# HasnainRaz/Fast-SRGAN

Measured on AMD Instinct MI355X. Metric: SR train-step images/sec (96->384 4x, full GAN step: G+D+VGG perceptual loss), higher is better.
Workload: dtype x3v; 1 GPU; BASELINE configs[2]: full GAN training step, 8 residual blocks / 64 filters, 96x96->384x384; per_gpu_batch=32, global_batch=32, parallelism=dp1, collectives=none, rccl_world_size=1, launch=hipGraph replay

## Files before the change

### fast-srgan_amd/csrc/conv_c3.hip

```cpp
#include "fsr_common.h"
#include "fsr_host.h"

namespace {

struct C3Args {
  const float* img;
  long long sn, sc, sh, sw;
  int N, H, W;
  float scale[3], shift[3];
  const void* wpk;
  const float* bias;
  const float* prelu;
  int act;
  float slope;
  int cout;
  void* out;
  void* preact;
  unsigned char* signs;
  const void* dz;
  float* ws;
  int tiles_x, tiles_y, tiles_per_slab, ntiles;
};

constexpr int PW = 18;
// ... 1 lines not shown
__device__ __forceinline__ int patch_off(int k) {
  const int tap = k / 3, ci = k - tap * 3;
  return ((tap / 3) * PW + (tap % 3)) * 3 + ci;
}

template <typename T> __device__ __forceinline__ float round_T(float v);
template <> __device__ __forceinline__ float round_T<float>(float v) { return v; }
template <> __device__ __forceinline__ float round_T<bf16_t>(float v) { return bf2f(f2bf(v)); }
template <> __device__ __forceinline__ float round_T<f16_t>(float v) { return (float)(f16_t)v; }

template <typename T, int TH>
__device__ __forceinline__ void stage_patch(const C3Args& a, float* patch, int n, int y0, int x0, int tid) {
  constexpr int PN = (TH + 2) * PW * 3;
  constexpr int PPT = (PN + 255) / 256;
  const float* src = a.img + n * a.sn;
  float v[PPT];
  unsigned okmask = 0u;
#pragma unroll
  for (int j = 0; j < PPT; ++j) {
    const int i = tid + j * 256;
    const int ci = i % 3, p = i / 3;
    const int px = p % PW, py = p / PW;
    const int y = y0 - 1 + py, x = x0 - 1 + px;
    const bool ok = i < PN && y >= 0 && y < a.H && x >= 0 && x < a.W;
    okmask |= (ok ? 1u : 0u) << j;
    v[j] = src[ok ? ci * a.sc + y * a.sh + x * a.sw : 0];
  }
#pragma unroll
  for (int j = 0; j < PPT; ++j) {
    const int i = tid + j * 256;
    const int ci = i % 3;
    const float sc = ci == 0 ? a.scale[0] : (ci == 1 ? a.scale[1] : a.scale[2]);
    const float sh = ci == 0 ? a.shift[0] : (ci == 1 ? a.shift[1] : a.shift[2]);
    if (i < PN) patch[i] = ((okmask >> j) & 1u) ? round_T<T>(v[j] * sc + sh) : 0.f;
  }
}

template <typename T, typename ST = T>
__global__ __launch_bounds__(256) void conv_c3_fwd_kernel(const C3Args a) {
  constexpr int TH = 16;
  __shared__ float patch[(TH + 2) * PW * 3];
  const int tid = threadIdx.x, lane = tid & 63, wave = __builtin_amdgcn_readfirstlane(tid >> 6);
  const int l15 = lane & 15, lg = lane >> 4;
  int bid = blockIdx.x;
  const int tx = bid % a.tiles_x;
  bid /= a.tiles_x;
  const int ty = bid % a.tiles_y;
  const int n = bid / a.tiles_y;
  const int nb = blockIdx.y;
  const int ntile = (a.cout - nb * 64 >= 64) ? 4 : (a.cout - nb * 64) / 16;
  stage_patch<T, TH>(a, patch, n, ty * TH, tx * 16, tid);

  const T* wpk = (const T*)a.wpk;
  int koff[8];
  if constexpr (sizeof(T) == 2) {
#pragma unroll
    for (int e = 0; e < 8; ++e) koff[e] = (8 * lg + e < 27) ? patch_off(8 * lg + e) : -1;
  } else {
#pragma unroll
    for (int j = 0; j < 8; ++j) koff[j] = (lg + 4 * j < 27) ? patch_off(lg + 4 * j) : -1;
  }
  constexpr bool X3 = std::is_same<ST, x3_t>::value;
  const bool wide = (sizeof(T) == 2 || X3) && ntile == 4;
  s16x8 wf16[4];
  float wf32[4][8];
#pragma unroll
  for (int t = 0; t < 4; ++t) {
    if (t < ntile) {
      const int ch = wide ? (t >> 1) * 32 + (l15 >> 2) * 8 + (t & 1) * 4 + (l15 & 3) : t * 16 + l15;
      const T* row = wpk + (size_t)(nb * 64 + ch) * 32;
      if constexpr (sizeof(T) == 2) {
        wf16[t] = *(const s16x8*)(row + 8 * lg);
      } else {
#pragma unroll
        for (int j = 0; j < 8; ++j) wf32[t][j] = row[lg + 4 * j];
      }
    }
  }
  float slope = (a.act == FSR_ACT_PRELU) ? a.prelu[0] : a.slope;
  if (a.act == FSR_ACT_NONE) slope = 1.f;
  if (a.act == FSR_ACT_RELU) slope = 0.f;
  __syncthreads();

  ST* outp = (ST*)a.out;
  ST* prep = (ST*)a.preact;
  const int gx = tx * 16 + l15;
  f32x4 bv[4];
#pragma unroll
  for (int i = 0; i < 4; ++i) bv[i] = (f32x4){0.f, 0.f, 0.f, 0.f};
  if (a.bias) {
    if (wide) {
#pragma unroll
      for (int p = 0; p < 2; ++p) {
        bv[2 * p] = *(const f32x4*)(a.bias + nb * 64 + p * 32 + lg * 8);
        bv[2 * p + 1] = *(const f32x4*)(a.bias + nb * 64 + p * 32 + lg * 8 + 4);
      }
    } else {
#pragma unroll
      for (int t = 0; t < 4; ++t)
        if (t < ntile) bv[t] = *(const f32x4*)(a.bias + nb * 64 + t * 16 + lg * 4);
    }
  }
#pragma unroll
  for (int m = 0; m < 4; ++m) {
    const int r = wave * 4 + m;
    const int gy = ty * TH + r;
    const float* base = patch + (r * PW + l15) * 3;
    float xv[8];
#pragma unroll
    for (int e = 0; e < 8; ++e) xv[e] = koff[e] >= 0 ? base[koff[e]] : 0.f;
    s16x8 xf16;
    if constexpr (sizeof(T) == 2) {
      const unsigned p0 = pack2<T>(xv[0], xv[1]), p1 = pack2<T>(xv[2], xv[3]);
      const unsigned p2 = pack2<T>(xv[4], xv[5]), p3 = pack2<T>(xv[6], xv[7]);
      xf16 = __builtin_bit_cast(s16x8, (u32x4){p0, p1, p2, p3});
    }
    if constexpr (sizeof(T) == 2) {
      if (wide) {
        f32x4 acc[4];
#pragma unroll
        for (int t = 0; t < 4; ++t) acc[t] = mfma16<T>(wf16[t], xf16, (f32x4){0.f, 0.f, 0.f, 0.f});
        if (gx < a.W && gy < a.H) {
          const size_t off = (((size_t)n * a.H + gy) * a.W + gx) * a.cout + nb * 64 + lg * 8;
#pragma unroll
          for (int p = 0; p < 2; ++p) {
            f32x4 lo = acc[2 * p], hi = acc[2 * p + 1];
            lo += bv[2 * p];
            hi += bv[2 * p + 1];
            if (prep)
              fsr_st<4>((u32x4*)((T*)prep + off + p * 32), (u32x4)((u32x4){pack2<T>(lo[0], lo[1]), pack2<T>(lo[2], lo[3]),
                                                       pack2<T>(hi[0], hi[1]), pack2<T>(hi[2], hi[3])}));
#pragma unroll
            for (int q = 0; q < 4; ++q) {
              lo[q] = fmaxf(lo[q], 0.f) + slope * fminf(lo[q], 0.f);
              hi[q] = fmaxf(hi[q], 0.f) + slope * fminf(hi[q], 0.f);
            }
            const u32x4 pk = (u32x4){pack2<T>(lo[0], lo[1]), pack2<T>(lo[2], lo[3]), pack2<T>(hi[0], hi[1]), pack2<T>(hi[2], hi[3])};
            fsr_st<4>((u32x4*)((T*)outp + off + p * 32), pk);
            if (a.signs) {
              unsigned b = 0u;
#pragma unroll
              for (int q = 0; q < 4; ++q) b |= ((int)(pk[q] << 16) > 0 ? 1u << (2 * q) : 0u) | ((int)(pk[q] & 0xffff0000u) > 0 ? 2u << (2 * q) : 0u);
              a.signs[(((size_t)n * a.H + gy) * a.W + gx) * (a.cout >> 3) + nb * 8 + p * 4 + lg] = (unsigned char)b;
            }
          }
        }
        continue;
      }
    }
    if constexpr (X3) {
      if (wide) {
        f32x4 acc[4];
#pragma unroll
        for (int t = 0; t < 4; ++t) {
          acc[t] = (f32x4){0.f, 0.f, 0.f, 0.f};
#pragma unroll
          for (int j = 0; j < 8; ++j) acc[t] = mfma_f32_16x16x4(wf32[t][j], xv[j], acc[t]);
        }
        if (gx < a.W && gy < a.H) {
          const size_t off = (((size_t)n * a.H + gy) * a.W + gx) * a.cout + nb * 64 + lg * 8;
#pragma unroll
          for (int p = 0; p < 2; ++p) {
            const f32x4 lo = acc[2 * p] + bv[2 * p], hi = acc[2 * p + 1] + bv[2 * p + 1];
            float v8[8] = {lo[0], lo[1], lo[2], lo[3], hi[0], hi[1], hi[2], hi[3]};
            if (prep) V16<x3_t, 4>::st((x3_t*)prep + off + p * 32, v8);
#pragma unroll
            for (int q = 0; q < 8; ++q) v8[q] = fmaxf(v8[q], 0.f) + slope * fminf(v8[q], 0.f);
            V16<x3_t, 4>::st((x3_t*)outp + off + p * 32, v8);
          }
        }
        continue;
      }
    }
    static_for<0, 4>([&](auto tc) {
      constexpr int t = decltype(tc)::value;
      if (t < ntile) {
        f32x4 acc = (f32x4){0.f, 0.f, 0.f, 0.f};
        if constexpr (sizeof(T) == 2) {
          acc = mfma16<T>(wf16[t], xf16, acc);
        } else {
#pragma unroll
          for (int j = 0; j < 8; ++j) acc = mfma_f32_16x16x4(wf32[t][j], xv[j], acc);
        }
        if (gx < a.W && gy < a.H) {
          const int co = nb * 64 + t * 16 + lg * 4;
          const size_t off = (((size_t)n * a.H + gy) * a.W + gx) * a.cout + co;
          acc += bv[t];
          if constexpr (sizeof(T) == 2) {
            if (prep) {
              u32x2 pk;
              pk.x = pack2<T>(acc[0], acc[1]);
              pk.y = pack2<T>(acc[2], acc[3]);
              fsr_st<4>((u32x2*)((T*)prep + off), (u32x2)(pk));
            }
          } else if constexpr (std::is_same<ST, x3_t>::value) {
            if (prep) x3_st4(prep + off, acc);
          } else {
            if (prep) *(f32x4*)(prep + off) = acc;
          }
#pragma unroll
          for (int q = 0; q < 4; ++q) acc[q] = fmaxf(acc[q], 0.f) + slope * fminf(acc[q], 0.f);
          if constexpr (sizeof(T) == 2) {
            u32x2 pk;
            pk.x = pack2<T>(acc[0], acc[1]);
            pk.y = pack2<T>(acc[2], acc[3]);
            fsr_st<4>((u32x2*)((T*)outp + off), (u32x2)(pk));
          } else if constexpr (std::is_same<ST, x3_t>::value) {
            x3_st4(outp + off, acc);
          } else {
            *(f32x4*)(outp + off) = acc;
          }
        }
      }
    });
  }
}

template <typename T, typename ST = T>
__global__ __launch_bounds__(256) void conv_c3_wgrad_kernel(const C3Args a) {
  constexpr int TH = 8;
  constexpr int PA = 64 + 16;
  __shared__ float patch[(TH + 2) * PW * 3];
  __shared__ __attribute__((aligned(16))) T dzt[TH * 16 * PA];
  const int tid = threadIdx.x, lane = tid & 63, wave = __builtin_amdgcn_readfirstlane(tid >> 6);
  const int l15 = lane & 15, lg = lane >> 4;
  const int slab = blockIdx.x, nb = blockIdx.y;
  const int cvalid = a.cout - nb * 64;
  const bool active = wave * 16 < cvalid;
  const ST* dzg = (const ST*)a.dz;
  constexpr int EPB = 16 / (int)sizeof(T);
  constexpr bool X3 = std::is_same<ST, x3_t>::value;

  const int off0 = patch_off(l15), off1 = (16 + l15 < 27) ? patch_off(16 + l15) : -1;
  const float ones27 = (l15 == 11) ? 1.f : 0.f;
  f32x4 acc0 = (f32x4){0.f, 0.f, 0.f, 0.f}, acc1 = (f32x4){0.f, 0.f, 0.f, 0.f};

  const int t0 = slab * a.tiles_per_slab;
  const int t1 = (t0 + a.tiles_per_slab < a.ntiles) ? t0 + a.tiles_per_slab : a.ntiles;
  for (int tile = t0; tile < t1; ++tile) {
    const int tx = tile % a.tiles_x;
    const int ty = (tile / a.tiles_x) % a.tiles_y;
    const int n = tile / (a.tiles_x * a.tiles_y);
    __syncthreads();
    stage_patch<T, TH>(a, patch, n, ty * TH, tx * 16, tid);
    if constexpr (X3) {
      constexpr int DU = TH * 16 * 8, DPT = DU / 256;
      u32x4 dh[DPT], dl[DPT];
#pragma unroll
      for (int j = 0; j < DPT; ++j) {
        const int u = tid + j * 256;
        const int unit = u % 8, p = u / 8;
        const int y = ty * TH + p / 16, x = tx * 16 + (p & 15);
        const bool ok = y < a.H && x < a.W && unit * 8 < cvalid;
        const char* hp = (const char*)x3_hi_ptr(dzg + (ok ? (((size_t)n * a.H + y) * a.W + x) * a.cout + nb * 64 + unit * 8 : 0));
        const u32x4 th = *(const u32x4*)hp, tl = *(const u32x4*)(hp + 64);
        dh[j] = ok ? th : (u32x4){0u, 0u, 0u, 0u};
        dl[j] = ok ? tl : (u32x4){0u, 0u, 0u, 0u};
      }
#pragma unroll
      for (int j = 0; j < DPT; ++j) {
        const int u = tid + j * 256;
        float* d = (float*)dzt + (u / 8) * PA + (u % 8) * 8;
        *(f32x4*)d = (f32x4){x3_join_lo(dh[j][0], dl[j][0]), x3_join_hi(dh[j][0], dl[j][0]), x3_join_lo(dh[j][1], dl[j][1]), x3_join_hi(dh[j][1], dl[j][1])};
        *(f32x4*)(d + 4) = (f32x4){x3_join_lo(dh[j][2], dl[j][2]), x3_join_hi(dh[j][2], dl[j][2]), x3_join_lo(dh[j][3], dl[j][3]), x3_join_hi(dh[j][3], dl[j][3])};
      }
    } else {
      constexpr int DU = TH * 16 * (64 / EPB), DPT = DU / 256;
      static_assert(DU % 256 == 0, "dz tile units per thread");
      u32x4 dv[DPT];
#pragma unroll
      for (int j = 0; j < DPT; ++j) {
        const int u = tid + j * 256;
        const int unit = u % (64 / EPB), p = u / (64 / EPB);
        const int y = ty * TH + p / 16, x = tx * 16 + (p & 15);
        const bool ok = y < a.H && x < a.W && unit * EPB < cvalid;
        const u32x4 t = *(const u32x4*)((const T*)dzg + (ok ? (((size_t)n * a.H + y) * a.W + x) * a.cout + nb * 64 + unit * EPB : 0));
        dv[j] = ok ? t : (u32x4){0u, 0u, 0u, 0u};
      }
#pragma unroll
      for (int j = 0; j < DPT; ++j) {
        const int u = tid + j * 256;
        *(u32x4*)(dzt + (u / (64 / EPB)) * PA + (u % (64 / EPB)) * EPB) = dv[j];
      }
    }
    __syncthreads();
    if (!active) continue;
    if constexpr (sizeof(T) == 2) {
      const int qrow = l15 >> 2, qch = (l15 & 3) * 4;
#pragma unroll
      for (int s = 0; s < TH / 2; ++s) {
        const int r = 2 * s + (lg >> 1), c0 = 8 * (lg & 1);
        const T* pa = dzt + (r * 16 + c0 + qrow) * PA + wave * 16 + qch;
        const s16x4 lo = __builtin_amdgcn_ds_read_tr16_b64_v4i16(FSR_LDS_PTR(s16x4, pa));
        const s16x4 hi = __builtin_amdgcn_ds_read_tr16_b64_v4i16(FSR_LDS_PTR(s16x4, pa + 4 * PA));
        const s16x8 af = (s16x8){lo[0], lo[1], lo[2], lo[3], hi[0], hi[1], hi[2], hi[3]};
        const float* pb = patch + (r * PW + c0) * 3;
        float b0[8], b1[8];
#pragma unroll
        for (int e = 0; e < 8; ++e) {
          b0[e] = pb[e * 3 + off0];
          b1[e] = off1 >= 0 ? pb[e * 3 + off1] : ones27;
        }
        const s16x8 bf0 = __builtin_bit_cast(s16x8, (u32x4){pack2<T>(b0[0], b0[1]), pack2<T>(b0[2], b0[3]),
                                                           pack2<T>(b0[4], b0[5]), pack2<T>(b0[6], b0[7])});
        const s16x8 bf1 = __builtin_bit_cast(s16x8, (u32x4){pack2<T>(b1[0], b1[1]), pack2<T>(b1[2], b1[3]),
                                                           pack2<T>(b1[4], b1[5]), pack2<T>(b1[6], b1[7])});
        acc0 = mfma16<T>(af, bf0, acc0);
        acc1 = mfma16<T>(af, bf1, acc1);
      }
    } else {
#pragma unroll 4
      for (int s = 0; s < TH * 4; ++s) {
        const int r = s >> 2, c = 4 * (s & 3) + lg;
        const float av = dzt[(r * 16 + c) * PA + wave * 16 + l15];
        const float* pb = patch + (r * PW + c) * 3;
        acc0 = mfma_f32_16x16x4(av, pb[off0], acc0);
        acc1 = mfma_f32_16x16x4(av, off1 >= 0 ? pb[off1] : ones27, acc1);
      }
    }
  }
  if (!active) return;
  float* o = a.ws + ((size_t)slab * a.cout + nb * 64 + wave * 16 + lg * 4) * 32 + l15;
#pragma unroll
  for (int r = 0; r < 4; ++r) {
    o[r * 32] = acc0[r];
    o[r * 32 + 16] = acc1[r];
  }
}

__global__ __launch_bounds__(256) void conv_c3_wgrad_reduce_kernel(const float* __restrict__ ws, float* __restrict__ dw, int nslab,
                                                                   int cout, float* __restrict__ dbias, int transposed) {
  __shared__ float red[8][32];
  const int total = cout * 32;
  const int k = threadIdx.x & 31, pl = threadIdx.x >> 5;
  const int co = blockIdx.x;
  const int i = co * 32 + k;
  float s = 0.f;
  const bool live = k < 27 || (k == 27 && dbias);
  if (live) {
    int j = pl;
    for (; j + 24 < nslab; j += 32) {
      const float v0 = ws[(size_t)j * total + i], v1 = ws[(size_t)(j + 8) * total + i];
      const float v2 = ws[(size_t)(j + 16) * total + i], v3 = ws[(size_t)(j + 24) * total + i];
      s = ((s + v0) + v1) + v2 + v3;
    }
    for (; j < nslab; j += 8) s += ws[(size_t)j * total + i];
  }
  red[pl][k] = s;
  __syncthreads();
  if (pl == 0 && live) {
    float r = red[0][k];
#pragma unroll
    for (int j = 1; j < 8; ++j) r += red[j][k];
    const int tap = k / 3, ci = k - tap * 3;
    float* o = (k == 27) ? dbias + co : (transposed ? dw + ((size_t)ci * cout + co) * 9 + (8 - tap) : dw + ((size_t)co * 3 + ci) * 9 + tap);
    *o += r;
  }
}

template <typename T>
__global__ void pack_c3_kernel(const float* __restrict__ w, T* __restrict__ out, int cout, int rows_pad, int transposed) {
  for (int i = blockIdx.x * blockDim.x + threadIdx.x; i < rows_pad * 32; i += gridDim.x * blockDim.x) {
    const int k = i & 31, row = i >> 5;
    float v = 0.f;
    if (row < cout && k < 27) {
      const int tap = k / 3, ci = k - tap * 3;
      v = transposed ? w[((size_t)ci * cout + row) * 9 + (8 - tap)] : w[((size_t)row * 3 + ci) * 9 + tap];
// ... 6 lines not shown
              long long sw, int n, int h, int w, const float (&scale3)[3], const float (&shift3)[3], int cout) {
  if (dtype != FSR_F32 && dtype != FSR_BF16 && dtype != FSR_F16 && dtype != FSR_X3) return fsr_fail(-2, "%s: unknown dtype %d", what, dtype);
  if (dtype == FSR_X3 && cout % 32) return fsr_fail(-2, "%s: x3 tensors have a multiple of 32 channels", what);
  if (!img) return fsr_fail(-1, "%s: null image", what);
  if (n <= 0 || h <= 0 || w <= 0) return fsr_fail(-2, "%s: bad dims", what);
  if (cout <= 0 || cout % 16) return fsr_fail(-2, "%s: cout=%d is not a multiple of 16", what, cout);
  if ((long long)n * h * w * cout >= (1LL << 31)) return fsr_fail(-2, "%s: tensors with 2^31 or more elements are not supported", what);
  a.img = img;
  a.sn = sn; a.sc = sc; a.sh = sh; a.sw = sw;
  a.N = n; a.H = h; a.W = w;
  for (int i = 0; i < 3; ++i) {
    a.scale[i] = scale3[i];
    a.shift[i] = shift3[i];
  }
  a.cout = cout;
  return 0;
}

}

extern "C" int fsr_pack_conv3x3_c3(int dtype, const float* w_oihw, int cout, void* packed, int transposed, fsr_stream_t stream_) {
  if (!w_oihw || !packed || cout <= 0) return fsr_fail(-1, "fsr_pack_conv3x3_c3: bad argument");
  const int rows_pad = (cout + 15) / 16 * 16;
  const int blocks = (rows_pad * 32 + 255) / 256;
  if (dtype == FSR_BF16)
    hipLaunchKernelGGL(pack_c3_kernel<bf16_t>, dim3(blocks), dim3(256), 0, (hipStream_t)stream_, w_oihw, (bf16_t*)packed, cout, rows_pad, transposed);
  else if (dtype == FSR_F16)
    hipLaunchKernelGGL(pack_c3_kernel<f16_t>, dim3(blocks), dim3(256), 0, (hipStream_t)stream_, w_oihw, (f16_t*)packed, cout, rows_pad, transposed);
  else if (dtype == FSR_F32 || dtype == FSR_X3)
    hipLaunchKernelGGL(pack_c3_kernel<float>, dim3(blocks), dim3(256), 0, (hipStream_t)stream_, w_oihw, (float*)packed, cout, rows_pad, transposed);
  else
    return fsr_fail(-2, "fsr_pack_conv3x3_c3: unknown dtype %d", dtype);
  return fsr_check_launch("pack_c3_kernel");
}

extern "C" int fsr_conv3x3_c3_fwd(int dtype, const float* img, long long sn, long long sc, long long sh, long long sw, int n,
                                  int h, int w, float scale0, float scale1, float scale2, float shift0, float shift1,
                                  float shift2, const void* packed_w, const float* bias, int act, float slope, const float* prelu_weight, int cout, void* out,
                                  void* preact, void* signs, fsr_stream_t stream_) {
  C3Args a = {};
  const float scale3[3] = {scale0, scale1, scale2}, shift3[3] = {shift0, shift1, shift2};
  if (int rc = fill_args(a, "fsr_conv3x3_c3_fwd", dtype, img, sn, sc, sh, sw, n, h, w, scale3, shift3, cout)) return rc;
  if (!packed_w || !out) return fsr_fail(-1, "fsr_conv3x3_c3_fwd: null argument");
  if (act == FSR_ACT_PRELU && !prelu_weight) return fsr_fail(-1, "fsr_conv3x3_c3_fwd: PReLU needs its weight");
  if (act == FSR_ACT_TANH) return fsr_fail(-2, "fsr_conv3x3_c3_fwd: tanh is not a first-layer activation");
  a.wpk = packed_w;
  a.bias = bias;
  a.prelu = prelu_weight;
  a.act = act;
  a.slope = slope;
  a.out = out;
  a.preact = preact;
  if (dtype == FSR_X3 && ((((size_t)out | (size_t)preact) & 127) != 0)) return fsr_fail(-2, "fsr_conv3x3_c3_fwd: x3 tensors must be 128-byte aligned");
  if (signs && (dtype == FSR_F32 || dtype == FSR_X3 || cout % 64 != 0)) return fsr_fail(-2, "fsr_conv3x3_c3_fwd: sign bits are written by the 16-bit kernels for cout %% 64 == 0");
  a.signs = (unsigned char*)signs;
  a.tiles_x = (w + 15) / 16;
  a.tiles_y = (h + 15) / 16;
  const long long nwg = (long long)a.tiles_x * a.tiles_y * n;
  if (nwg > 0x7fffffffLL) return fsr_fail(-2, "fsr_conv3x3_c3_fwd: bad grid");
  const dim3 grid((unsigned)nwg, (unsigned)((cout + 63) / 64));
  if (dtype == FSR_BF16) hipLaunchKernelGGL(conv_c3_fwd_kernel<bf16_t>, grid, dim3(256), 0, (hipStream_t)stream_, a);
  else if (dtype == FSR_F16) hipLaunchKernelGGL(conv_c3_fwd_kernel<f16_t>, grid, dim3(256), 0, (hipStream_t)stream_, a);
  else if (dtype == FSR_X3) hipLaunchKernelGGL((conv_c3_fwd_kernel<float, x3_t>), grid, dim3(256), 0, (hipStream_t)stream_, a);
  else hipLaunchKernelGGL(conv_c3_fwd_kernel<float>, grid, dim3(256), 0, (hipStream_t)stream_, a);
  return fsr_check_launch("conv_c3_fwd_kernel");
}

static int c3_wgrad_slabs(int n, int h, int w, int* tiles_x, int* tiles_y, int* per) {
  *tiles_x = (w + 15) / 16;
  *tiles_y = (h + 7) / 8;
  const long long ntiles = (long long)*tiles_x * *tiles_y * n;
  long long want = 1024;
  if (want > ntiles) want = ntiles;
  *per = (int)((ntiles + want - 1) / want);
  return (int)((ntiles + *per - 1) / *per);
}

extern "C" size_t fsr_conv3x3_c3_wgrad_workspace(int n, int h, int w, int cout) {
  int tx, ty, per;
  if (n <= 0 || h <= 0 || w <= 0 || cout <= 0) return 0;
  return (size_t)c3_wgrad_slabs(n, h, w, &tx, &ty, &per) * cout * 32 * sizeof(float);
}

extern "C" int fsr_conv3x3_c3_wgrad(int dtype, const float* img, long long sn, long long sc, long long sh, long long sw,
                                    int n, int h, int w, float scale0, float scale1, float scale2, float shift0,
                                    float shift1, float shift2, const void* dz, int cout, float* dw_oihw, float* dbias, void* workspace, int transposed,
                                    fsr_stream_t stream_) {
  C3Args a = {};
  const float scale3[3] = {scale0, scale1, scale2}, shift3[3] = {shift0, shift1, shift2};
  if (int rc = fill_args(a, "fsr_conv3x3_c3_wgrad", dtype, img, sn, sc, sh, sw, n, h, w, scale3, shift3, cout)) return rc;
  if (!dz || !dw_oihw || !workspace) return fsr_fail(-1, "fsr_conv3x3_c3_wgrad: null argument");
  if (dtype == FSR_X3 && (((size_t)dz & 127) != 0)) return fsr_fail(-2, "fsr_conv3x3_c3_wgrad: x3 tensors must be 128-byte aligned");
  a.dz = dz;
  a.ws = (float*)workspace;
  const int nslab = c3_wgrad_slabs(n, h, w, &a.tiles_x, &a.tiles_y, &a.tiles_per_slab);
  a.ntiles = a.tiles_x * a.tiles_y * n;
  const dim3 grid((unsigned)nslab, (unsigned)((cout + 63) / 64));
  if (dtype == FSR_BF16) hipLaunchKernelGGL(conv_c3_wgrad_kernel<bf16_t>, grid, dim3(256), 0, (hipStream_t)stream_, a);
  else if (dtype == FSR_F16) hipLaunchKernelGGL(conv_c3_wgrad_kernel<f16_t>, grid, dim3(256), 0, (hipStream_t)stream_, a);
  else if (dtype == FSR_X3) hipLaunchKernelGGL((conv_c3_wgrad_kernel<float, x3_t>), grid, dim3(256), 0, (hipStream_t)stream_, a);
  else hipLaunchKernelGGL(conv_c3_wgrad_kernel<float>, grid, dim3(256), 0, (hipStream_t)stream_, a);
  if (int rc = fsr_check_launch("conv_c3_wgrad_kernel")) return rc;
  hipLaunchKernelGGL(conv_c3_wgrad_reduce_kernel, dim3(cout), dim3(256), 0, (hipStream_t)stream_, (const float*)workspace,
                     dw_oihw, nslab, cout, dbias, transposed);
  return fsr_check_launch("conv_c3_wgrad_reduce_kernel");
}
```

### fast-srgan_amd/csrc/conv_s2d3.hip

```cpp
#include "fsr_common.h"
#include "fsr_conv_args.h"
#include "fsr_host.h"

#include <stdlib.h>

#ifndef FSR_ABLS
#define FSR_ABLS 0
#endif

namespace {

constexpr int S2D_ABL = FSR_ABLS;

typedef float f32x16 __attribute__((ext_vector_type(16)));

template <typename T> struct Mfma32;
template <> struct Mfma32<bf16_t> {
  static __device__ __forceinline__ f32x16 run(s16x8 a, s16x8 b, f32x16 c) {
    return __builtin_amdgcn_mfma_f32_32x32x16_bf16(__builtin_bit_cast(bf16x8_hw, a), __builtin_bit_cast(bf16x8_hw, b), c, 0, 0, 0);
  }
};
template <> struct Mfma32<f16_t> {
  static __device__ __forceinline__ f32x16 run(s16x8 a, s16x8 b, f32x16 c) {
    return __builtin_amdgcn_mfma_f32_32x32x16_f16(__builtin_bit_cast(f16x8_hw, a), __builtin_bit_cast(f16x8_hw, b), c, 0, 0, 0);
// ... 343 lines not shown
          if (ok1) fsr_st<16>((u32x4*)((T*)outp + off1), o1);
        }
        }
      });
    });
    if (!has_nxt) break;
    cur = nxt;
#pragma unroll
    for (int k = 0; k < HPW; ++k) hv_cur[k] = hv_nxt[k];
    ws_cur = ws_nxt;
    tile = next;
    next = tile + nround;
    has_nxt = next < a.t3_ntiles;
    acc_zero();
  }
}

int s2d_cus() {
  if (const char* e = getenv("FSR_PERSIST_CUS")) {
    const int v = atoi(e);
    if (v > 0) return v;
  }
  static int cus = 0;
  if (cus == 0) {
    int dev = 0;
    hipDeviceProp_t prop;
    cus = (hipGetDevice(&dev) == hipSuccess && hipGetDeviceProperties(&prop, dev) == hipSuccess && prop.multiProcessorCount > 0)
              ? prop.multiProcessorCount : 256;
  }
  return cus;
}

template <typename T, bool X3 = false>
int s2d_launch(ConvKArgs& a, hipStream_t stream) {
  auto kern = conv_s2d3_kernel<T, X3>;
  static bool attr_set = false;
  if (!attr_set) {
    (void)hipFuncSetAttribute((const void*)kern, hipFuncAttributeMaxDynamicSharedMemorySize, S2D_LDS);
    attr_set = true;
  }
  long long grid = (long long)s2d_cus() * 2;
  if (grid > a.t3_ntiles) grid = a.t3_ntiles;
  hipLaunchKernelGGL(kern, dim3((unsigned)grid), dim3(S2D_NW * 64), S2D_LDS, stream, a);
  fsr_note_kernel("conv_s2d3_kernel<%s>", X3 ? "x3" : (std::is_same<T, f16_t>::value ? "f16" : "bf16"));
  const int rc = fsr_check_launch("conv_s2d3_kernel");
  return rc ? rc : 1;
}

}

int fsr_conv_s2d3_try(int dtype, ConvKArgs& a, hipStream_t stream) {
  static const bool off = getenv("FSR_S2D3") && atoi(getenv("FSR_S2D3")) == 0;
  if (off || (dtype != FSR_BF16 && dtype != FSR_F16 && dtype != FSR_X3)) return 0;
  if (dtype == FSR_X3 && ((a.Cin & 63) != 0 || (a.Cin >> 6) * 3 >= (1 << 15) || a.dmask_bits)) return 0;
  if (a.Cin < 64 || a.Cin % 32 != 0 || a.Cout % 64 != 0 || a.Cout < 64 || a.CoutPad != a.Cout) return 0;
  if (a.ps || a.in_ps || a.out_f32 || a.preact || a.oscale || a.bias || a.stats || a.pool2 || a.act != FSR_ACT_NONE || a.dmask_add) return 0;
  if (a.IH != (a.FOH - 1) / 2 + 1 || a.IW != (a.FOW - 1) / 2 + 1) return 0;
  if ((long long)a.N * a.IH * a.IW * a.Cin >= (1LL << 31) || (long long)a.N * a.FOH * a.FOW * a.Cout >= (1LL << 31)) return 0;
  ConvKArgs b = a;
  b.tiles_x = (b.IW + 15) / 16;
  b.tiles_y = (b.IH + S2D_TH - 1) / S2D_TH;
  b.nblk_n = b.Cout / S2D_BN;
  const long long ntiles = (long long)b.tiles_x * b.tiles_y * b.N * b.nblk_n;
  if (ntiles <= 0 || ntiles > 0x7fffffffLL) return 0;
  b.t3_ntiles = (int)ntiles;
  const int want = b.Cin >= 128 ? S2D_BN : 0;
  if (b.query) {
    a.wlin_want = want;
    return 1;
  }
  if (b.wlin != 0 && b.wlin != S2D_BN)
    return fsr_fail(-2, "conv_s2d3: the filter pack is stage-contiguous in blocks of %d channels, this launch needs %d", b.wlin, S2D_BN);
  for (int t = 0; t < 9; ++t) b.t3_woff[t] = b.wlin ? (unsigned)(t * S2D_BN * 64) : (unsigned)((size_t)t * b.CoutPad * b.Cin * 2);
  const int rc = dtype == FSR_X3 ? s2d_launch<bf16_t, true>(b, stream) : (dtype == FSR_F16 ? s2d_launch<f16_t>(b, stream) : s2d_launch<bf16_t>(b, stream));
  if (rc == 1) a = b;
  return rc;
}
```

### fast-srgan_amd/csrc/fsr_api.hip

```cpp
#include <string.h>

#include "fsr_common.h"
#include "fsr_conv_args.h"
#include "fsr_host.h"

static thread_local char g_err[512] = "";

int fsr_fail(int code, const char* fmt, ...) {
  va_list ap;
  va_start(ap, fmt);
  vsnprintf(g_err, sizeof(g_err), fmt, ap);
  va_end(ap);
  return code;
}

int fsr_check_launch(const char* what) {
  hipError_t e = hipGetLastError();
  if (e != hipSuccess) return fsr_fail(-3, "%s: launch failed: %s", what, hipGetErrorString(e));
  return 0;
}

static thread_local char g_kernel[160] = "";

void fsr_note_kernel(const char* fmt, ...) {
// ... 31 lines not shown
static int conv3x3_enqueue(const fsr_conv_desc* d, ConvKArgs& a, hipStream_t stream);

static int conv3x3_impl(const fsr_conv_desc* d, const void* in, const void* packed_w, const float* bias,
                        const float* prelu_weight, const float* oscale, const void* dact_mask, float dact_slope,
                        void* out, void* preact, float* stats, void* scratch, hipStream_t stream, int* query_block);

extern "C" int fsr_conv3x3(const fsr_conv_desc* d, const void* in, const void* packed_w, const float* bias,
                           const float* prelu_weight, const float* oscale, const void* dact_mask, float dact_slope,
                           void* out, void* preact, float* stats, void* scratch, fsr_stream_t stream_) {
  return conv3x3_impl(d, in, packed_w, bias, prelu_weight, oscale, dact_mask, dact_slope, out, preact, stats, scratch,
                      (hipStream_t)stream_, nullptr);
}

extern "C" int fsr_conv3x3_pack_block(const fsr_conv_desc* d, int optional_tensors) {
  if (!d) return fsr_fail(-1, "fsr_conv3x3_pack_block: null descriptor");
  static const float dummy_f[4] = {0.f, 0.f, 0.f, 0.f};
  const void* some = dummy_f;
  fsr_conv_desc q = *d;
  q.pack_lin = 0;
  int block = 0;
  const int rc = conv3x3_impl(&q, some, some, (optional_tensors & FSR_OPT_BIAS) ? dummy_f : nullptr,
                              (optional_tensors & FSR_OPT_PRELU) ? dummy_f : nullptr, (optional_tensors & FSR_OPT_OSCALE) ? dummy_f : nullptr,
                              (optional_tensors & FSR_OPT_MASK) ? some : nullptr, 0.f, (void*)some,
                              (optional_tensors & FSR_OPT_PREACT) ? (void*)some : nullptr,
                              (optional_tensors & FSR_OPT_STATS) ? (float*)some : nullptr,
                              (optional_tensors & FSR_OPT_STATS) ? (void*)some : nullptr, nullptr, &block);
  return rc < 0 ? rc : block;
}

static int conv3x3_impl(const fsr_conv_desc* d, const void* in, const void* packed_w, const float* bias,
                        const float* prelu_weight, const float* oscale, const void* dact_mask, float dact_slope,
                        void* out, void* preact, float* stats, void* scratch, hipStream_t stream, int* query_block) {
  if (!d || !in || !packed_w || !out) return fsr_fail(-1, "fsr_conv3x3: null argument");
  if (stats && !scratch) return fsr_fail(-1, "fsr_conv3x3: statistics need the scratch buffer (fsr_conv3x3_scratch bytes)");
  if (d->stride != 1 && d->stride != 2) return fsr_fail(-2, "fsr_conv3x3: stride must be 1 or 2");
  if (d->act == FSR_ACT_PRELU && !prelu_weight) return fsr_fail(-1, "fsr_conv3x3: PReLU needs its weight");
  if (d->n <= 0 || d->ih <= 0 || d->iw <= 0 || d->oh <= 0 || d->ow <= 0) return fsr_fail(-2, "fsr_conv3x3: bad dims");

  ConvKArgs a;
  memset(&a, 0, sizeof(a));
  a.in = in;
  a.wpk = packed_w;
  a.out = out;
  a.bias = bias;
  a.prelu = prelu_weight;
  a.preact = preact;
  a.oscale = oscale;
  a.dmask = dact_mask;
  a.dmask_slope = dact_slope;
  a.dmask_add = (dact_mask && d->mask_is_addend == 1) ? 1 : 0;
  a.dmask_bits = (dact_mask && d->mask_is_addend == 2) ? 1 : 0;
  if (d->mask_is_addend && !dact_mask) return fsr_fail(-1, "fsr_conv3x3: mask_is_addend needs the dact_mask tensor");
  if (d->mask_is_addend < 0 || d->mask_is_addend > 2) return fsr_fail(-2, "fsr_conv3x3: mask_is_addend must be 0, 1 or 2");
  if (a.dmask_bits && (d->mode != FSR_CONV_DGRAD || d->stride != 2 || d->dtype == FSR_F32 || d->dtype == FSR_X3 || d->cout % 64 != 0))
    return fsr_fail(-2, "fsr_conv3x3: a sign-bit mask (mask_is_addend = 2) is read by the stride-2 data gradients of the 16-bit modes, cout %% 64 == 0");
  a.stats = stats ? (float*)scratch : nullptr;
  a.stats_P_max = stats ? (int)stats_slots_bound(d) : 0;
  a.query = query_block ? 1 : 0;
  a.wlin = d->pack_lin;
  if (d->pack_lin != 0 && d->pack_lin != 64 && d->pack_lin != 128) return fsr_fail(-2, "fsr_conv3x3: pack_lin must be 0, 64 or 128");
  a.N = d->n;
  a.IH = d->ih;
  a.IW = d->iw;
  a.Cin = d->dtype == FSR_X3 ? 2 * d->cin : d->cin;
  a.Cout = d->cout;
  if (d->dtype == FSR_X3) {
    if (d->cin % 32 != 0) return fsr_fail(-2, "fsr_conv3x3: x3 tensors have a multiple of 32 channels (cin = %d)", d->cin);
    if (!d->out_f32 && d->cout % 32 != 0) return fsr_fail(-2, "fsr_conv3x3: x3 tensors have a multiple of 32 channels (cout = %d)", d->cout);
    if (d->pixel_shuffle && (d->cout / 4) % 32 != 0) return fsr_fail(-2, "fsr_conv3x3: x3 pixel shuffle needs cout / 4 %% 32 == 0");
    if (d->in_pixel_shuffled && (d->cin / 4) % 32 != 0) return fsr_fail(-2, "fsr_conv3x3: x3 in_pixel_shuffled needs cin / 4 %% 32 == 0");
    if (!query_block && ((((size_t)in | (d->out_f32 ? 0 : (size_t)out) | (size_t)preact | (size_t)dact_mask) & 127) != 0))
      return fsr_fail(-2, "fsr_conv3x3: x3 tensors must be 128-byte aligned");
  }
  a.CoutPad = (d->cout + 15) / 16 * 16;
  a.FOH = d->oh;
  a.FOW = d->ow;
  a.act = d->act;
  a.slope = d->slope;
  a.ps = d->pixel_shuffle;
  a.in_ps = d->in_pixel_shuffled;
  a.out_f32 = d->out_f32;
  a.pool2 = d->pool2;
  if (d->pool2 && (d->mode != FSR_CONV_FWD || d->dtype == FSR_F32 || d->stride != 1 || d->pixel_shuffle || d->out_f32 || stats || preact ||
                   dact_mask || oscale || (d->oh & 1) || (d->ow & 1) || d->cout % 16 != 0 || d->act == FSR_ACT_TANH))
    return fsr_fail(-2, "fsr_conv3x3: pool2 is for stride-1 forward launches of the 16-bit modes with even output extents "
                        "(no statistics / pre-activation / mask / scale tensors, no pixel shuffle)");
  if (d->out_f32 < 0 || d->out_f32 > FSR_OUT_I420) return fsr_fail(-2, "fsr_conv3x3: unknown output kind %d", d->out_f32);
  if (d->out_f32 == FSR_OUT_U8 && (d->act != FSR_ACT_TANH || d->cout > 16 || d->pixel_shuffle || d->mode != FSR_CONV_FWD))
    return fsr_fail(-2, "fsr_conv3x3: uint8 image output is for tanh heads (forward, cout <= 16)");
  if (d->out_f32 == FSR_OUT_I420) {
    if (d->act != FSR_ACT_TANH || d->cout != 3 || d->pixel_shuffle || d->mode != FSR_CONV_FWD || d->stride != 1 || stats || preact ||
        dact_mask || oscale)
      return fsr_fail(-2, "fsr_conv3x3: I420 output is for 3-channel tanh heads (forward, stride 1, no pixel shuffle, no statistics / "
                          "pre-activation / mask / scale tensors)");
    if ((d->oh & 1) || (d->ow & 1)) return fsr_fail(-2, "fsr_conv3x3: I420 output needs even output extents (%d x %d)", d->oh, d->ow);
    if ((d->yuv_matrix != FSR_YUV_BT601 && d->yuv_matrix != FSR_YUV_BT709) || (d->yuv_full_range != 0 && d->yuv_full_range != 1))
      return fsr_fail(-2, "fsr_conv3x3: I420 output: unknown colour matrix %d / range %d", d->yuv_matrix, d->yuv_full_range);
  }
  a.yuv_matrix = d->yuv_matrix;
  a.yuv_full = d->yuv_full_range;
  if (a.ps && stats) return fsr_fail(-2, "fsr_conv3x3: statistics are not available together with pixel shuffle");
  if ((stats || preact || dact_mask) && (d->cout % 16 != 0 || (d->out_f32 && d->dtype != FSR_F32)))
    return fsr_fail(-2, "fsr_conv3x3: statistics / pre-activation / mask tensors need cout %% 16 == 0 and a `dtype` output");
  if (a.ps && (d->cout % 16 != 0)) return fsr_fail(-2, "fsr_conv3x3: pixel shuffle needs cout %% 16 == 0");
  if (a.in_ps && (d->cin % 4 != 0)) return fsr_fail(-2, "fsr_conv3x3: in_pixel_shuffled needs cin %% 4 == 0");
  if (stats && d->mode == FSR_CONV_DGRAD && d->stride != 1)
    return fsr_fail(-2, "fsr_conv3x3: statistics are not available for stride-2 data gradients");

  if (int rc = conv3x3_enqueue(d, a, stream)) return rc;
  if (query_block) {
    *query_block = a.wlin_want;
    return 0;
  }
  if (stats) {
    return fsr_launch_reduce_partials((const float*)scratch, stats, d->n, a.stats_P, d->cout * 2, d->cout * 2, a.stats_tpi, a.stats_per, 1.f, 0, stream);
  }
  return 0;
}

static int conv3x3_enqueue(const fsr_conv_desc* d, ConvKArgs& a, hipStream_t stream) {
  if (d->mode == FSR_CONV_FWD) {
    if (d->oh != (d->ih - 1) / d->stride + 1 || d->ow != (d->iw - 1) / d->stride + 1)
      return fsr_fail(-2, "fsr_conv3x3: output dims do not match k=3,p=1,stride=%d", d->stride);
    a.GH = d->oh;
// ... 75 lines not shown
```

### fast-srgan_amd/ops.py

```python
import ctypes
import os
import weakref

import torch

from . import _lib as L

_DT = {"f32": (L.FSR_F32, torch.float32, 16), "bf16": (L.FSR_BF16, torch.bfloat16, 32), "f16": (L.FSR_F16, torch.float16, 32),
       "x3": (L.FSR_X3, torch.float32, 32)}


class Compute:

    def __init__(self, name="f16"):
        if name not in _DT:
            raise ValueError("compute dtype must be 'bf16', 'f16', 'x3' or 'f32', got %r" % (name,))
        self.name = name
        self.code, self.torch_dtype, self.cpad = _DT[name]
        self.x3 = name == "x3"
        self.pack_dtype = torch.bfloat16 if self.x3 else self.torch_dtype
        self.pack_kmul = 2 if self.x3 else 1
        self.is16 = name in ("bf16", "f16")

    def pad(self, c):
# ... 431 lines not shown
    prof = PROFILE_CONV
    if prof is not None:
        ev0, ev1 = torch.cuda.Event(enable_timing=True), torch.cuda.Event(enable_timing=True)
        ev0.record()
    L.check(L.lib().fsr_conv3x3_wgrad(ctypes.byref(d), _p(x), _p(dy), _p(dw), _p(ws), _stream()), "fsr_conv3x3_wgrad")
    if prof is not None:
        ev1.record()
        nbytes = x.numel() * x.element_size() + dy.numel() * dy.element_size() + cout * cin * 9 * 4
        prof.append((ev0, ev1, 2.0 * n * oh * ow * cout * cin * 9, nbytes, "conv_wgrad_kernel", "wgrad"))
    return dw


def image_to_nhwc(cd, img, scale=(1.0, 1.0, 1.0), shift=(0.0, 0.0, 0.0)):
    _check_dev(img)
    if img.dtype != torch.float32:
        img = img.float()
    n, c, h, w = img.shape
    if c != 3:
        raise ValueError("expected a 3-channel image batch, got %s" % (tuple(img.shape),))
    out = _empty((n, h, w, cd.cpad), cd.torch_dtype, img.device)
    sn, sc, sh, sw = img.stride()
    L.check(L.lib().fsr_image_to_nhwc(cd.code, _p(img), sn, sc, sh, sw, n, h, w, scale[0], scale[1], scale[2], shift[0],
                                      shift[1], shift[2], _p(out), cd.cpad, _stream()), "fsr_image_to_nhwc")
    return out


class ConvCfg:

    def __init__(self, cd, *, stride=1, act=L.ACT_NONE, slope=0.0, pixel_shuffle=False, stats=False, image_in=False,
                 in_scale=(1.0, 1.0, 1.0), in_shift=(0.0, 0.0, 0.0), tanh_head=False, input_act_bwd=None,
                 act_bwd_by_consumer=False, u8_head=False, pool_after=False, n_alias=0, emit_signs=False, i420_head=None):
        self.input_act_bwd, self.act_bwd_by_consumer = input_act_bwd, act_bwd_by_consumer
        self.cd, self.stride, self.act, self.slope = cd, stride, act, slope
        self.pixel_shuffle, self.stats, self.image_in = pixel_shuffle, stats, image_in
        self.in_scale, self.in_shift, self.tanh_head = in_scale, in_shift, tanh_head
        self.u8_head = u8_head and tanh_head
        self.i420_head = i420_head if tanh_head else None
        self.pool_after = pool_after
        self.n_alias = n_alias
        self.emit_signs = emit_signs


class Conv3x3Fn(torch.autograd.Function):

    @staticmethod
    def forward(ctx, x, weight, bias, prelu, cfg, grad_on=True):
        ctx.grad_on = grad_on
        cd = cfg.cd
        cout, cin = weight.shape[0], weight.shape[1]
        if (cfg.image_in and cfg.stride == 1 and cout % 16 == 0 and not (cfg.pixel_shuffle or cfg.stats or cfg.tanh_head)
                and USE_C3_KERNELS):
            return Conv3x3Fn._forward_c3(ctx, x, weight, bias, prelu, cfg)
        ctx.c3 = False
        ctx.in_signs = getattr(x, "_fsr_signs", None) if (cfg.input_act_bwd is not None and cfg.stride == 2 and cd.is16) else None
        if cfg.image_in:
            xin = image_to_nhwc(cd, x, cfg.in_scale, cfg.in_shift)
        else:
            xin = x if x.is_contiguous() else x.contiguous()
            if xin.dtype != cd.torch_dtype:
                raise L.FsrError("activation dtype %s does not match the module's compute dtype %s" % (xin.dtype, cd.name))
        cin_pad = xin.shape[3]
        wpk = FilterSpec(weight, L.PACK_FWD_PS if cfg.pixel_shuffle else L.PACK_FWD, cin_pad)
        training = ctx.grad_on and any(ctx.needs_input_grad)
        if (cfg.u8_head or cfg.i420_head or cfg.pool_after) and training:
            raise L.FsrError("the uint8 / I420 head and fused max-pool epilogues are inference-only: they have no gradient")
        act = L.ACT_TANH if cfg.tanh_head else cfg.act
        want_pre = training and act == L.ACT_PRELU
        b32 = bias if bias is None or bias.dtype == torch.float32 else bias.float()
        out, pre, stats = conv3x3_raw(cd, xin, wpk, cout, stride=cfg.stride, bias=b32, act=act, slope=cfg.slope,
                                      prelu=prelu, pixel_shuffle=cfg.pixel_shuffle, out_f32=cfg.tanh_head,
                                      want_stats=cfg.stats, want_preact=want_pre, alg_k=cin, out_u8=cfg.u8_head,
                                      pool2=cfg.pool_after, out_i420=cfg.i420_head)
        ctx.cfg = cfg
        ctx.dims = (cout, cin, tuple(xin.shape))
        ctx.has_bias = bias is not None
        ctx.x_is_image = cfg.image_in
        saved_act = pre if want_pre else (out if act in (L.ACT_RELU, L.ACT_LEAKY, L.ACT_TANH) else None)
        ctx.save_for_backward(xin, weight, prelu, saved_act)
        if stats is None:
            stats = torch.empty(0, device=out.device)
        ctx.mark_non_differentiable(stats)
        ctx.set_materialize_grads(False)
        if cfg.u8_head or cfg.i420_head:
            return out, stats
        if cfg.tanh_head:
            return out.permute(0, 3, 1, 2), stats
        if cfg.n_alias:
            if cfg.image_in or cfg.input_act_bwd is not None or cfg.pixel_shuffle or cfg.stride != 1:
                raise L.FsrError("skip aliases are for plain stride-1 convolutions on NHWC activations")
            return (out, stats) + tuple(xin.view_as(xin) for _ in range(cfg.n_alias))
        return out, stats

    @staticmethod
    def _forward_c3(ctx, x, weight, bias, prelu, cfg):
        cd = cfg.cd
        _check_dev(x)
        if x.dtype != torch.float32:
            x = x.float()
        n, c, h, w = x.shape
        if c != 3:
            raise ValueError("expected a 3-channel image batch, got %s" % (tuple(x.shape),))
        cout = weight.shape[0]
        wpk = packed_filter(cd, weight, PACK_C3, 32)
        training = ctx.grad_on and any(ctx.needs_input_grad)
        want_pre = training and cfg.act == L.ACT_PRELU
        b32 = bias if bias is None or bias.dtype == torch.float32 else bias.float()
        out = _empty((n, h, w, cout), cd.torch_dtype, x.device)
        pre = _empty_like(out) if want_pre else None
        signs = (torch.empty((n, h, w, cout // 8), dtype=torch.uint8, device=x.device)
                 if (cfg.emit_signs and USE_SIGN_BITS and training and cd.is16 and cout % 64 == 0) else None)
        sn, sc, sh, sw = x.stride()
        prof = PROFILE_CONV
        if prof is not None:
            ev0, ev1 = torch.cuda.Event(enable_timing=True), torch.cuda.Event(enable_timing=True)
            ev0.record()
        L.check(L.lib().fsr_conv3x3_c3_fwd(cd.code, _p(x), sn, sc, sh, sw, n, h, w, *cfg.in_scale, *cfg.in_shift, _p(wpk),
                                           _p(b32), cfg.act, float(cfg.slope), _p(prelu), cout, _p(out), _p(pre), _p(signs), _stream()),
                "fsr_conv3x3_c3_fwd")
        if signs is not None:
            out._fsr_signs = signs
        if prof is not None:
            ev1.record()
            nbytes = x.numel() * 4 + out.numel() * out.element_size() * (2 if want_pre else 1) + wpk.numel() * wpk.element_size()
            prof.append((ev0, ev1, 2.0 * n * h * w * cout * 27, nbytes, "conv_c3_fwd_kernel", "fwd"))
        ctx.cfg = cfg
        ctx.c3 = True
        ctx.bias_param = bias
        ctx.dims = (cout, 3, (n, h, w, cd.cpad))
        ctx.has_bias = bias is not None
        ctx.x_is_image = True
        saved_act = pre if want_pre else (out if cfg.act in (L.ACT_RELU, L.ACT_LEAKY) else None)
        ctx.save_for_backward(x, weight, prelu, saved_act)
        stats = torch.empty(0, device=out.device)
        ctx.mark_non_differentiable(stats)
        ctx.set_materialize_grads(False)
        return out, stats

    @staticmethod
    def backward(ctx, g, _gstats, *g_alias):
        skips = [t for t in g_alias if t is not None]
        if g is None:
            dx = None
            for t in skips:
                dx = t if dx is None else add(ctx.cfg.cd, dx, t)
            return dx, None, None, None, None, None
        cfg, cd = ctx.cfg, ctx.cfg.cd
        xin, weight, prelu, saved = ctx.saved_tensors
        cout, cin, xshape = ctx.dims
        n, ih, iw, cin_pad = xshape
        lib, st = L.lib(), _stream()
        dbias = _zeros((cout,), xin.device) if ctx.has_bias else None
        dprelu = None
        act = L.ACT_TANH if cfg.tanh_head else cfg.act
        if cfg.tanh_head and USE_C3_KERNELS and cout == 3 and cin_pad % 16 == 0 and cin == cin_pad:
            return Conv3x3Fn._backward_head_c3(ctx, g)
        if cfg.tanh_head:
            if g.dtype != torch.float32:
                g = g.float()
            _, _, h, w = g.shape
            dz = _empty((n, h, w, cd.cpad), cd.torch_dtype, xin.device)
            sn, sc, sh, sw = g.stride()
            L.check(lib.fsr_tanh_bwd_to_nhwc(cd.code, _p(g), sn, sc, sh, sw, _p(saved), n, h, w, _p(dz), cd.cpad, _p(dbias),
                                             _p(_workspace(lib.fsr_tanh_bwd_scratch(), xin.device)), st), "fsr_tanh_bwd_to_nhwc")
# ... 470 lines not shown
```

Before: 613.0 images/s.

## Enable sign-bit masks for x3, trim c3 K loop, swizzle wgrad LDS, size grid by CUs

Extends the sign-bit activation mask path to the x3 dtype: the c3 forward kernel now emits packed sign bits from the hi words, and the stride-2 dgrad plus the s2d3 fast path accept sign-bit masks for x3. This lets the discriminator's first layer avoid reading the full activation mask. The fp32/x3 c3 forward drops the always-zero eighth K slice, cutting one MFMA per tile. The wgrad kernel replaces LDS row padding with an XOR swizzle for fp32, and its slab count now comes from the CU count times occupancy instead of a fixed 1024. The swizzle and grid sizing could change LDS conflicts and load balance in either direction.

New measurement: 617.2 images/s (median of 6 runs). Within noise of the previous version (+0.7%).

```diff
diff --git a/fast-srgan_amd/csrc/conv_c3.hip b/fast-srgan_amd/csrc/conv_c3.hip
--- a/fast-srgan_amd/csrc/conv_c3.hip
+++ b/fast-srgan_amd/csrc/conv_c3.hip
@@ -77,18 +77,19 @@
   stage_patch<T, TH>(a, patch, n, ty * TH, tx * 16, tid);
 
   const T* wpk = (const T*)a.wpk;
-  int koff[8];
+  constexpr int KS = sizeof(T) == 2 ? 8 : 7;
+  int koff[KS];
   if constexpr (sizeof(T) == 2) {
 #pragma unroll
     for (int e = 0; e < 8; ++e) koff[e] = (8 * lg + e < 27) ? patch_off(8 * lg + e) : -1;
   } else {
 #pragma unroll
-    for (int j = 0; j < 8; ++j) koff[j] = (lg + 4 * j < 27) ? patch_off(lg + 4 * j) : -1;
+    for (int j = 0; j < KS; ++j) koff[j] = (lg + 4 * j < 27) ? patch_off(lg + 4 * j) : -1;
   }
   constexpr bool X3 = std::is_same<ST, x3_t>::value;
   const bool wide = (sizeof(T) == 2 || X3) && ntile == 4;
   s16x8 wf16[4];
-  float wf32[4][8];
+  float wf32[4][KS];
 #pragma unroll
   for (int t = 0; t < 4; ++t) {
     if (t < ntile) {
@@ -98,7 +99,7 @@
         wf16[t] = *(const s16x8*)(row + 8 * lg);
       } else {
 #pragma unroll
-        for (int j = 0; j < 8; ++j) wf32[t][j] = row[lg + 4 * j];
+        for (int j = 0; j < KS; ++j) wf32[t][j] = row[lg + 4 * j];
       }
     }
   }
@@ -131,9 +132,9 @@
     const int r = wave * 4 + m;
     const int gy = ty * TH + r;
     const float* base = patch + (r * PW + l15) * 3;
-    float xv[8];
-#pragma unroll
-    for (int e = 0; e < 8; ++e) xv[e] = koff[e] >= 0 ? base[koff[e]] : 0.f;
+    float xv[KS];
+#pragma unroll
+    for (int e = 0; e < KS; ++e) xv[e] = koff[e] >= 0 ? base[koff[e]] : 0.f;
     s16x8 xf16;
     if constexpr (sizeof(T) == 2) {
       const unsigned p0 = pack2<T>(xv[0], xv[1]), p1 = pack2<T>(xv[2], xv[3]);
@@ -180,7 +181,7 @@
         for (int t = 0; t < 4; ++t) {
           acc[t] = (f32x4){0.f, 0.f, 0.f, 0.f};
 #pragma unroll
-          for (int j = 0; j < 8; ++j) acc[t] = mfma_f32_16x16x4(wf32[t][j], xv[j], acc[t]);
+          for (int j = 0; j < KS; ++j) acc[t] = mfma_f32_16x16x4(wf32[t][j], xv[j], acc[t]);
         }
         if (gx < a.W && gy < a.H) {
           const size_t off = (((size_t)n * a.H + gy) * a.W + gx) * a.cout + nb * 64 + lg * 8;
@@ -191,7 +192,23 @@
             if (prep) V16<x3_t, 4>::st((x3_t*)prep + off + p * 32, v8);
 #pragma unroll
             for (int q = 0; q < 8; ++q) v8[q] = fmaxf(v8[q], 0.f) + slope * fminf(v8[q], 0.f);
-            V16<x3_t, 4>::st((x3_t*)outp + off + p * 32, v8);
+            u32x4 hw, lw;
+#pragma unroll
+            for (int q = 0; q < 4; ++q) {
+              unsigned h2, l2;
+              x3_split2(v8[2 * q], v8[2 * q + 1], h2, l2);
+              hw[q] = h2;
+              lw[q] = l2;
+            }
+            char* hp = (char*)x3_hi_ptr((x3_t*)outp + off + p * 32);
+            fsr_st<4>((u32x4*)hp, hw);
+            fsr_st<4>((u32x4*)(hp + 64), lw);
+            if (a.signs) {
+              unsigned b = 0u;
+#pragma unroll
+              for (int q = 0; q < 4; ++q) b |= ((int)(hw[q] << 16) > 0 ? 1u << (2 * q) : 0u) | ((int)(hw[q] & 0xffff0000u) > 0 ? 2u << (2 * q) : 0u);
+              a.signs[(((size_t)n * a.H + gy) * a.W + gx) * (a.cout >> 3) + nb * 8 + p * 4 + lg] = (unsigned char)b;
+            }
           }
         }
         continue;
@@ -205,7 +222,7 @@
           acc = mfma16<T>(wf16[t], xf16, acc);
         } else {
 #pragma unroll
-          for (int j = 0; j < 8; ++j) acc = mfma_f32_16x16x4(wf32[t][j], xv[j], acc);
+          for (int j = 0; j < KS; ++j) acc = mfma_f32_16x16x4(wf32[t][j], xv[j], acc);
         }
         if (gx < a.W && gy < a.H) {
           const int co = nb * 64 + t * 16 + lg * 4;
@@ -244,7 +261,7 @@
 template <typename T, typename ST = T>
 __global__ __launch_bounds__(256) void conv_c3_wgrad_kernel(const C3Args a) {
   constexpr int TH = 8;
-  constexpr int PA = 64 + 16;
+  constexpr int PA = sizeof(T) == 2 ? 64 + 16 : 64;
   __shared__ float patch[(TH + 2) * PW * 3];
   __shared__ __attribute__((aligned(16))) T dzt[TH * 16 * PA];
   const int tid = threadIdx.x, lane = tid & 63, wave = __builtin_amdgcn_readfirstlane(tid >> 6);
@@ -285,7 +302,7 @@
 #pragma unroll
       for (int j = 0; j < DPT; ++j) {
         const int u = tid + j * 256;
-        float* d = (float*)dzt + (u / 8) * PA + (u % 8) * 8;
+        float* d = (float*)dzt + (u / 8) * PA + (((u % 8) * 8) ^ (((u / 8) & 3) << 4));
         *(f32x4*)d = (f32x4){x3_join_lo(dh[j][0], dl[j][0]), x3_join_hi(dh[j][0], dl[j][0]), x3_join_lo(dh[j][1], dl[j][1]), x3_join_hi(dh[j][1], dl[j][1])};
         *(f32x4*)(d + 4) = (f32x4){x3_join_lo(dh[j][2], dl[j][2]), x3_join_hi(dh[j][2], dl[j][2]), x3_join_lo(dh[j][3], dl[j][3]), x3_join_hi(dh[j][3], dl[j][3])};
       }
@@ -305,7 +322,8 @@
 #pragma unroll
       for (int j = 0; j < DPT; ++j) {
         const int u = tid + j * 256;
-        *(u32x4*)(dzt + (u / (64 / EPB)) * PA + (u % (64 / EPB)) * EPB) = dv[j];
+        const int px = u / (64 / EPB), ch = (u % (64 / EPB)) * EPB;
+        *(u32x4*)(dzt + px * PA + (sizeof(T) == 2 ? ch : ch ^ ((px & 3) << 4))) = dv[j];
       }
     }
     __syncthreads();
@@ -337,7 +355,7 @@
 #pragma unroll 4
       for (int s = 0; s < TH * 4; ++s) {
         const int r = s >> 2, c = 4 * (s & 3) + lg;
-        const float av = dzt[(r * 16 + c) * PA + wave * 16 + l15];
+        const float av = dzt[(r * 16 + c) * PA + ((wave * 16 + l15) ^ ((c & 3) << 4))];
         const float* pb = patch + (r * PW + c) * 3;
         acc0 = mfma_f32_16x16x4(av, pb[off0], acc0);
         acc1 = mfma_f32_16x16x4(av, off1 >= 0 ? pb[off1] : ones27, acc1);
@@ -450,7 +468,7 @@
   a.out = out;
   a.preact = preact;
   if (dtype == FSR_X3 && ((((size_t)out | (size_t)preact) & 127) != 0)) return fsr_fail(-2, "fsr_conv3x3_c3_fwd: x3 tensors must be 128-byte aligned");
-  if (signs && (dtype == FSR_F32 || dtype == FSR_X3 || cout % 64 != 0)) return fsr_fail(-2, "fsr_conv3x3_c3_fwd: sign bits are written by the 16-bit kernels for cout %% 64 == 0");
+  if (signs && (dtype == FSR_F32 || cout % 64 != 0)) return fsr_fail(-2, "fsr_conv3x3_c3_fwd: sign bits are written by the 16-bit and x3 kernels for cout %% 64 == 0");
   a.signs = (unsigned char*)signs;
   a.tiles_x = (w + 15) / 16;
   a.tiles_y = (h + 15) / 16;
@@ -464,11 +482,52 @@
   return fsr_check_launch("conv_c3_fwd_kernel");
 }
 
-static int c3_wgrad_slabs(int n, int h, int w, int* tiles_x, int* tiles_y, int* per) {
+static int c3_cus() {
+  if (const char* e = getenv("FSR_PERSIST_CUS")) {
+    const int v = atoi(e);
+    if (v > 0) return v;
+  }
+  static int cus = 0;
+  if (cus == 0) {
+    int dev = 0;
+    hipDeviceProp_t prop;
+    cus = (hipGetDevice(&dev) == hipSuccess && hipGetDeviceProperties(&prop, dev) == hipSuccess && prop.multiProcessorCount > 0)
+              ? prop.multiProcessorCount : 256;
+  }
+  return cus;
+}
+
+constexpr int C3_WG_PER_CU = 4;
+
+template <typename T, typename ST>
+static int c3_wgrad_resident() {
+#ifdef FSR_EMU_BUILD
+  return C3_WG_PER_CU;
+#else
+  static int wgs = 0;
+  if (wgs == 0) {
+    int v = 0;
+    if (hipOccupancyMaxActiveBlocksPerMultiprocessor(&v, conv_c3_wgrad_kernel<T, ST>, 256, 0) != hipSuccess || v <= 0) v = C3_WG_PER_CU;
+    wgs = v < C3_WG_PER_CU ? v : C3_WG_PER_CU;
+  }
+  return wgs;
+#endif
+}
+
+static int c3_wgrad_resident(int dtype) {
+  if (dtype == FSR_BF16) return c3_wgrad_resident<bf16_t, bf16_t>();
+  if (dtype == FSR_F16) return c3_wgrad_resident<f16_t, f16_t>();
+  if (dtype == FSR_X3) return c3_wgrad_resident<float, x3_t>();
+  return c3_wgrad_resident<float, float>();
+}
+
+static int c3_wgrad_slabs(int n, int h, int w, int wg_per_cu, int* tiles_x, int* tiles_y, int* per) {
   *tiles_x = (w + 15) / 16;
   *tiles_y = (h + 7) / 8;
   const long long ntiles = (long long)*tiles_x * *tiles_y * n;
-  long long want = 1024;
+  static const int force = getenv("FSR_C3_WGRAD_WG") ? atoi(getenv("FSR_C3_WGRAD_WG")) : 0;
+  if (force >= 1 && force <= C3_WG_PER_CU) wg_per_cu = force;
+  long long want = (long long)c3_cus() * wg_per_cu;
   if (want > ntiles) want = ntiles;
   *per = (int)((ntiles + want - 1) / want);
   return (int)((ntiles + *per - 1) / *per);
@@ -477,7 +536,7 @@
 extern "C" size_t fsr_conv3x3_c3_wgrad_workspace(int n, int h, int w, int cout) {
   int tx, ty, per;
   if (n <= 0 || h <= 0 || w <= 0 || cout <= 0) return 0;
-  return (size_t)c3_wgrad_slabs(n, h, w, &tx, &ty, &per) * cout * 32 * sizeof(float);
+  return (size_t)c3_wgrad_slabs(n, h, w, C3_WG_PER_CU, &tx, &ty, &per) * cout * 32 * sizeof(float);
 }
 
 extern "C" int fsr_conv3x3_c3_wgrad(int dtype, const float* img, long long sn, long long sc, long long sh, long long sw,
@@ -491,7 +550,7 @@
   if (dtype == FSR_X3 && (((size_t)dz & 127) != 0)) return fsr_fail(-2, "fsr_conv3x3_c3_wgrad: x3 tensors must be 128-byte aligned");
   a.dz = dz;
   a.ws = (float*)workspace;
-  const int nslab = c3_wgrad_slabs(n, h, w, &a.tiles_x, &a.tiles_y, &a.tiles_per_slab);
+  const int nslab = c3_wgrad_slabs(n, h, w, c3_wgrad_resident(dtype), &a.tiles_x, &a.tiles_y, &a.tiles_per_slab);
   a.ntiles = a.tiles_x * a.tiles_y * n;
   const dim3 grid((unsigned)nslab, (unsigned)((cout + 63) / 64));
   if (dtype == FSR_BF16) hipLaunchKernelGGL(conv_c3_wgrad_kernel<bf16_t>, grid, dim3(256), 0, (hipStream_t)stream_, a);
diff --git a/fast-srgan_amd/csrc/conv_s2d3.hip b/fast-srgan_amd/csrc/conv_s2d3.hip
--- a/fast-srgan_amd/csrc/conv_s2d3.hip
+++ b/fast-srgan_amd/csrc/conv_s2d3.hip
@@ -419,7 +419,7 @@
 int fsr_conv_s2d3_try(int dtype, ConvKArgs& a, hipStream_t stream) {
   static const bool off = getenv("FSR_S2D3") && atoi(getenv("FSR_S2D3")) == 0;
   if (off || (dtype != FSR_BF16 && dtype != FSR_F16 && dtype != FSR_X3)) return 0;
-  if (dtype == FSR_X3 && ((a.Cin & 63) != 0 || (a.Cin >> 6) * 3 >= (1 << 15) || a.dmask_bits)) return 0;
+  if (dtype == FSR_X3 && ((a.Cin & 63) != 0 || (a.Cin >> 6) * 3 >= (1 << 15))) return 0;
   if (a.Cin < 64 || a.Cin % 32 != 0 || a.Cout % 64 != 0 || a.Cout < 64 || a.CoutPad != a.Cout) return 0;
   if (a.ps || a.in_ps || a.out_f32 || a.preact || a.oscale || a.bias || a.stats || a.pool2 || a.act != FSR_ACT_NONE || a.dmask_add) return 0;
   if (a.IH != (a.FOH - 1) / 2 + 1 || a.IW != (a.FOW - 1) / 2 + 1) return 0;
diff --git a/fast-srgan_amd/csrc/fsr_api.hip b/fast-srgan_amd/csrc/fsr_api.hip
--- a/fast-srgan_amd/csrc/fsr_api.hip
+++ b/fast-srgan_amd/csrc/fsr_api.hip
@@ -107,8 +107,8 @@
   a.dmask_bits = (dact_mask && d->mask_is_addend == 2) ? 1 : 0;
   if (d->mask_is_addend && !dact_mask) return fsr_fail(-1, "fsr_conv3x3: mask_is_addend needs the dact_mask tensor");
   if (d->mask_is_addend < 0 || d->mask_is_addend > 2) return fsr_fail(-2, "fsr_conv3x3: mask_is_addend must be 0, 1 or 2");
-  if (a.dmask_bits && (d->mode != FSR_CONV_DGRAD || d->stride != 2 || d->dtype == FSR_F32 || d->dtype == FSR_X3 || d->cout % 64 != 0))
-    return fsr_fail(-2, "fsr_conv3x3: a sign-bit mask (mask_is_addend = 2) is read by the stride-2 data gradients of the 16-bit modes, cout %% 64 == 0");
+  if (a.dmask_bits && (d->mode != FSR_CONV_DGRAD || d->stride != 2 || d->dtype == FSR_F32 || d->cout % 64 != 0))
+    return fsr_fail(-2, "fsr_conv3x3: a sign-bit mask (mask_is_addend = 2) is read by the stride-2 data gradients of the 16-bit and x3 modes, cout %% 64 == 0");
   a.stats = stats ? (float*)scratch : nullptr;
   a.stats_P_max = stats ? (int)stats_slots_bound(d) : 0;
   a.query = query_block ? 1 : 0;
@@ -124,7 +124,7 @@
     if (!d->out_f32 && d->cout % 32 != 0) return fsr_fail(-2, "fsr_conv3x3: x3 tensors have a multiple of 32 channels (cout = %d)", d->cout);
     if (d->pixel_shuffle && (d->cout / 4) % 32 != 0) return fsr_fail(-2, "fsr_conv3x3: x3 pixel shuffle needs cout / 4 %% 32 == 0");
     if (d->in_pixel_shuffled && (d->cin / 4) % 32 != 0) return fsr_fail(-2, "fsr_conv3x3: x3 in_pixel_shuffled needs cin / 4 %% 32 == 0");
-    if (!query_block && ((((size_t)in | (d->out_f32 ? 0 : (size_t)out) | (size_t)preact | (size_t)dact_mask) & 127) != 0))
+    if (!query_block && ((((size_t)in | (d->out_f32 ? 0 : (size_t)out) | (size_t)preact | (a.dmask_bits ? 0 : (size_t)dact_mask)) & 127) != 0))
       return fsr_fail(-2, "fsr_conv3x3: x3 tensors must be 128-byte aligned");
   }
   a.CoutPad = (d->cout + 15) / 16 * 16;
diff --git a/fast-srgan_amd/ops.py b/fast-srgan_amd/ops.py
--- a/fast-srgan_amd/ops.py
+++ b/fast-srgan_amd/ops.py
@@ -507,7 +507,7 @@
                 and USE_C3_KERNELS):
             return Conv3x3Fn._forward_c3(ctx, x, weight, bias, prelu, cfg)
         ctx.c3 = False
-        ctx.in_signs = getattr(x, "_fsr_signs", None) if (cfg.input_act_bwd is not None and cfg.stride == 2 and cd.is16) else None
+        ctx.in_signs = getattr(x, "_fsr_signs", None) if (cfg.input_act_bwd is not None and cfg.stride == 2 and (cd.is16 or cd.x3)) else None
         if cfg.image_in:
             xin = image_to_nhwc(cd, x, cfg.in_scale, cfg.in_shift)
         else:
@@ -563,7 +563,7 @@
         out = _empty((n, h, w, cout), cd.torch_dtype, x.device)
         pre = _empty_like(out) if want_pre else None
         signs = (torch.empty((n, h, w, cout // 8), dtype=torch.uint8, device=x.device)
-                 if (cfg.emit_signs and USE_SIGN_BITS and training and cd.is16 and cout % 64 == 0) else None)
+                 if (cfg.emit_signs and USE_SIGN_BITS and training and (cd.is16 or cd.x3) and cout % 64 == 0) else None)
         sn, sc, sh, sw = x.stride()
         prof = PROFILE_CONV
         if prof is not None:
```
